# python-microscopy/ch-shrinkwrap

Measured on AMD Instinct MI355X. Metric: vertex-updates/s (force+CG step) + achieved HBM GB/s, 1M pts/200k verts, higher is better.
Workload: dtype f32; 1 GPU; BASELINE configs[2]: two-lobe vesicle (smooth union of two R=300 nm spheres), 1000000 localizations sigma=10 nm, 198812 vertices / 397620 faces, lams=[10], blocks of 5 iterations, fixed topology; localizations_per_gpu=1000000, vertices_per_gpu=198812, faces_per_gpu=397620, block=5, mode=single, parallelism=single GPU

## Files before the change

ch_shrinkwrap_amd/build.py:

```python
import glob
import os
import subprocess

HERE = os.path.dirname(os.path.abspath(__file__))
LIB = os.path.join(HERE, 'libnanowrap_hip.so')


def _csrc(name):
    return os.path.join(HERE, 'csrc', name)


def _include(name):
    return os.path.join(os.path.dirname(HERE), 'include', name)


HIPCC_FLAGS = ['-O3', '--offload-arch=gfx950', '-fPIC', '-shared', '-ffp-contract=off', '-munsafe-fp-atomics',
               '-fvisibility=hidden', '-Wall', '-Wno-unused-function']
_BASE = ['-O3', '--offload-arch=gfx950', '-fPIC', '-fvisibility=hidden']
_QUERY = _BASE + ['-ffp-contract=off', '-Wall', '-Wno-unused-function']
_BQ = [_csrc('nw_bq.h'), _csrc('nw_device.h')]

OBJ_MAIN, OBJ_HOLEPUNCH, OBJ_SURGERY, OBJ_BQ = _csrc('nanowrap.o'), _csrc('nw_holepunch.o'), _csrc('nw_surgery.o'), _csrc('nw_bq.o')
OBJ_ISOSURFACE = _csrc('nw_isosurface.o')
OBJ_EVALUATION = _csrc('nw_evaluation.o')
# ... 17 lines not shown
def needs_build():
    if not os.path.exists(LIB):
        return True
    t = os.path.getmtime(LIB)
    return any(os.path.getmtime(d) > t for d in DEPS)


def build_hip_library(force=False, verbose=False):
    if not force and not needs_build():
        return LIB
    hipcc = os.environ.get('HIPCC', '/opt/rocm/bin/hipcc')

    def run(cmd):
        if verbose:
            print(' '.join(cmd))
        subprocess.check_call(cmd)

    for src, obj, extra, flags in UNITS:
        if force or not os.path.exists(obj) or os.path.getmtime(obj) < max(os.path.getmtime(d) for d in [src] + extra):
            run([hipcc] + flags + ['-c', '-o', obj, src])
    check_kernel_budgets(verbose=verbose)
    run([hipcc, '--offload-arch=gfx950', '-fPIC', '-shared', '-o', LIB] + [obj for _, obj, _, _ in UNITS])
    return LIB


LLVM_BIN = os.environ.get('NW_LLVM_BIN', '/opt/rocm/lib/llvm/bin')
KERNEL_BUDGETS = {
    'k_nn_wave<false>':               (80, 10 * 1024),
    'k_attract':                      (72, 20 * 1024),
    'k_face_centroids':               (64, 8 * 1024),
    'k_centroid_scatter':             (64, 0),
    'k_scan_final':                   (64, 1024),
    'k_prior_ring':                   (128, 1024),
    'k_prior_directions':             (96, 1024),
    'k_subspace_point_sums':          (128, 1024),
    'k_solve_update':                 (128, 1024),
    'k_hp_empty_faces':               (64, 0),
    'k_hp_pair':                      (64, 8 * 1024),
    'k_hp_prism':                     (176, 0),
    'k_hp_cell_count':                (32, 0),
    'k_hp_scatter':                   (32, 0),
    'k_hp_bbox':                      (32, 0),
    'k_hp_cand_geom':                 (32, 0),
    'k_hp_pair_final':                (16, 0),
    'k_ws_init':                      (16, 0),
    'k_ws_hook':                      (32, 0),
    'k_ws_compress':                  (16, 0),
    'k_ws_number':                    (16, 0),
    'k_ws_stats':                     (64, 0),
    'k_ws_bbox_init':                 (16, 0),
    'k_ws_active':                    (16, 0),
    'k_ws_winding':                   (176, 0),
    'k_ws_lengths':                   (16, 0),
    'k_ws_hist':                      (16, 2048),
    'k_ws_pick':                      (32, 0),
    'k_ws_flag':                      (16, 0),
    'k_iso_count':                    (16, 16 * 1024),
    'k_iso_widen':                    (16, 0),
    'k_iso_smooth':                   (16, 0),
    'k_iso_hist':                     (16, 1024),
    'k_iso_pattern':                  (32, 0),
    'k_iso_compact':                  (16, 0),
    'k_iso_cell_counts':              (16, 0),
    'k_iso_vertices':                 (64, 0),
    'k_iso_quads':                    (32, 0),
    'k_ev_face_setup':                (64, 0),
    'k_ev_node_test':                 (32, 0),
    'k_ev_emit':                      (32, 0),
    'k_ev_bbox':                      (48, 0),
# ... 101 lines not shown
```

ch_shrinkwrap_amd/csrc/nanowrap.hip:

```cpp
#include <hip/hip_runtime.h>
#include <cstdio>
#include <cstdlib>
#include <cstring>
#include <cmath>
#include <string>
#include <vector>
#include <algorithm>
#include <chrono>
#include <thread>
#include <mutex>
#include <condition_variable>
#include <functional>
#include <atomic>
#include <memory>

#include "../../include/nanowrap.h"
#include "nw_kernels.h"

int nw_sort_pairs_u32(const unsigned *key_in, unsigned *key_out, const int *val_in, int *val_out, int n, int bits, hipStream_t stream);

static_assert(sizeof(NwIterLogDev) == sizeof(nw_iter_log), "device/host log record mismatch");
static_assert(SC_COUNT <= NW_N_SCALARS, "scalar slots");

#define NW_EXPORT extern "C" __attribute__((visibility("default")))
// ... 1524 lines not shown
        hipLaunchKernelGGL(k_nn_fixup, dim3(fb), dim3(NW_BLOCK), 0, ctx->stream, g, ctx->ambig_list.p, ctx->ambig_count.p, ctx->pts.p, ctx->cstart.p, ctx->cent.p,
                           ctx->cent_tmp.p, ctx->face.p, ctx->state.p, it, ctx->face_sorted ? ctx->face_orig.p : nullptr);
    }
    NW_HIP(hipGetLastError());
    return NW_OK;
}

static int iter_attract_parts(nw_ctx *ctx, int parts)
{
    if (ctx->begin_ops_pending) NW_TRY(enqueue_begin_ops(ctx));
    const int it = ctx->search_done;
    const int64_t N = ctx->N;
    const bool attract_rides = (parts & QP_NN) && (parts & QP_ATTRACT) && attract_in_nn() && fuse_fixup() && ctx->item_done.p != nullptr && ctx->face_warm && !ctx->handoff_off;
    bool rode = false;
    if (parts & (QP_GRID | QP_NN | QP_FIXUP)) NW_TRY(launch_query(ctx, it, parts & (QP_GRID | QP_NN | QP_FIXUP), true, attract_rides, &rode));
    if ((parts & QP_ATTRACT) && !rode) {
        StageScope s(ctx, ST_ATTRACT);
        hipLaunchKernelGGL(k_attract, dim3(attract_blocks(ctx)), dim3(NW_BLOCK), 0, ctx->stream, (int)N, ctx->pts.p, ctx->face.p, attract_args(ctx), ctx->state.p, it);
        ctx->attract_rows = attract_blocks(ctx);
    }
    NW_HIP(hipGetLastError());
    return NW_OK;
}

NW_EXPORT int nw_iter_attract(nw_ctx *ctx)
{
    if (!ctx || !ctx->in_search) return fail(ctx, NW_ERR_BADARG, "nw_iter_attract outside a search");
    if (ctx->have_boundary && ctx->pos_unpack_pending) { ctx->pos_unpack_pending = false; NW_TRY(halo_unpack(ctx, NW_ARR_POS)); }
    NW_TRY(iter_attract_parts(ctx, QP_ALL));
    if (ctx->have_boundary) NW_TRY(halo_pack(ctx, NW_ARR_VACC));
    return NW_OK;
}

NW_EXPORT int nw_iter_directions(nw_ctx *ctx)
{
    if (!ctx || !ctx->in_search) return fail(ctx, NW_ERR_BADARG, "nw_iter_directions outside a search");
    if (ctx->have_boundary) NW_TRY(halo_unpack(ctx, NW_ARR_VACC));
    const int it = ctx->search_done;
    const int n_search = (ctx->search_done == 0 || (ctx->search_flags & NW_FLAG_NO_LAST_STEP)) ? 2 : 3;
    {
        StageScope s(ctx, ST_PRIOR);
        const bool wfunc = (ctx->search_flags & NW_FLAG_WFUNC) != 0;
        if (wfunc)
            hipLaunchKernelGGL(k_vertex_area_weights, dim3(nblk(ctx->M)), dim3(NW_BLOCK), 0, ctx->stream, (int)ctx->M, ctx->NB, ctx->nbr.p, ctx->pos.p, ctx->wv.p, ctx->state.p, it);
        if (!ring_in_nn()) hipLaunchKernelGGL(k_prior_ring, dim3(nblk(ctx->M)), dim3(NW_BLOCK), 0, ctx->stream, ring_args(ctx), ctx->state.p, it);
        hipLaunchKernelGGL(k_prior_directions, dim3(prior_blocks(ctx)), dim3(NW_BLOCK), 0, ctx->stream, (int)ctx->M, ctx->ring4.p, ctx->ring_a.p, ctx->pos.p,
                           ctx->meshpos.p, ctx->nrm.p, ctx->vacc.p, ctx->S.p, ctx->fdef.p, ctx->pi.p, ctx->part_p.p, ctx->state.p, it, n_search,
                           ctx->acc_quantum, ctx->w_quantum, wfunc ? ctx->wv.p : nullptr, ctx->have_owned ? ctx->owned.p : nullptr);
    }
    {
        StageScope s(ctx, ST_AS);
        hipLaunchKernelGGL(k_subspace_point_sums, dim3(subspace_blocks(ctx)), dim3(NW_BLOCK), 0, ctx->stream, (int)ctx->N, (int)ctx->M, ctx->vidx.p, ctx->w.p, ctx->res.p,
                           ctx->mask.p, ctx->S.p, ctx->part_s.p, ctx->state.p, it, n_search);
        hipLaunchKernelGGL(k_reduce_scalars, dim3(3 * NW_SPARTS), dim3(NW_BLOCK), 0, ctx->stream, ctx->part_a.p, ctx->attract_rows, ctx->part_p.p, prior_blocks(ctx),
                           ctx->part_s.p, subspace_blocks(ctx), ctx->scalars.p, ctx->state.p, it);
    }
    NW_HIP(hipGetLastError());
    return NW_OK;
}

NW_EXPORT int nw_iter_update(nw_ctx *ctx)
{
    if (!ctx || !ctx->in_search) return fail(ctx, NW_ERR_BADARG, "nw_iter_update outside a search");
    if (ctx->search_done >= ctx->search_iters) return fail(ctx, NW_ERR_BADARG, "nw_iter_update: more iterations than announced");
    const int it = ctx->search_done;
    const int n_search = (ctx->search_done == 0 || (ctx->search_flags & NW_FLAG_NO_LAST_STEP)) ? 2 : 3;
    {
        StageScope s(ctx, ST_UPDATE);
        hipLaunchKernelGGL(k_solve_update, dim3(std::min(nblk(ctx->M), 512)), dim3(NW_BLOCK), 0, ctx->stream, (int)ctx->M, ctx->lam0, n_search, ctx->search_flags,
                           ctx->have_valid ? ctx->valid.p : nullptr, ctx->pos.p, ctx->meshpos.p, ctx->S.p, ctx->vacc.p, ctx->scalars.p, ctx->state.p,
                           ctx->logs.p + ctx->search_done, it, (ctx->direct_out && it == ctx->search_iters - 1) ? (float *)ctx->pin : nullptr);
    }
    NW_HIP(hipGetLastError());
    if (ctx->have_boundary) { NW_TRY(halo_pack(ctx, NW_ARR_POS)); ctx->pos_unpack_pending = true; }
    ctx->global_iter += 1;
    ctx->search_done += 1;
    return NW_OK;
}

static int write_back_impl(nw_ctx *ctx, float *contiguous, void *rows, int64_t row_stride_bytes);
static int ensure_staging(nw_ctx *ctx);
static void copy_out_staged(nw_ctx *ctx, float *contiguous, void *rows, int64_t row_stride_bytes);
static bool copy_out_chunks(nw_ctx *ctx, float *contiguous, void *rows, int64_t row_stride_bytes, int64_t slice_rows, int flag_base);

static int ensure_pin_log(nw_ctx *ctx, int n_records)
{
    const size_t log_bytes = (size_t)std::max(n_records, 1) * sizeof(nw_iter_log);
    if (ctx->pin_log_bytes < log_bytes + sizeof(NwDevState)) {
        if (ctx->pin_log) (void)hipHostFree(ctx->pin_log);
        ctx->pin_log = nullptr; ctx->pin_log_bytes = 0;
        NW_HIP(hipHostMalloc(&ctx->pin_log, 2 * log_bytes + sizeof(NwDevState), hipHostMallocDefault));
        ctx->pin_log_bytes = 2 * log_bytes + sizeof(NwDevState);
    }
    return NW_OK;
}

static bool spin_wait_on() { static const bool on = !(getenv("NW_SPIN_WAIT") && atoi(getenv("NW_SPIN_WAIT")) == 0); return on; }
static int enqueue_block_done(nw_ctx *ctx)
{
    ctx->done_launched = false;
    if (!spin_wait_on() || ctx->search_done <= 0) return NW_OK;
    NW_TRY(ensure_pin_log(ctx, ctx->search_iters));
    if (!ctx->pin_flag) {
        NW_HIP(hipHostMalloc((void **)&ctx->pin_flag, 64, hipHostMallocDefault));
        ctx->pin_flag[0] = 0;
        NW_HIP(ctx->done_count.ensure(1));
        NW_HIP(hipMemsetAsync(ctx->done_count.p, 0, sizeof(int), ctx->stream));
        ctx->done_expected = 0;
    }
    NwDevState *stp = (NwDevState *)((char *)ctx->pin_log + ctx->pin_log_bytes - sizeof(NwDevState));
// ... 274 lines not shown
    if (r == ncclSuccess) r = e;
    if (r != ncclSuccess) return fail(ctx, NW_ERR_HIP, std::string("ncclSend/ncclRecv: ") + (g_rccl.GetErrorString ? g_rccl.GetErrorString(r) : "error"));
    return NW_OK;
}

static int comm_after_attract(nw_ctx *ctx)
{
    if (!ctx->comm || !ctx->comm_mode) return NW_OK;
    if (ctx->comm_mode & NW_FLAG_COMM_REPLICATED) return comm_all_reduce_dev(ctx, ctx->vacc.p, (size_t)4 * ctx->M, ncclInt64, ncclSum);
    if ((ctx->comm_mode & NW_FLAG_COMM_HALO) && ctx->have_boundary && ctx->have_peers) {
        NW_TRY(px_exchange(ctx, false, 4, ncclInt64, 8));
        NW_TRY(px_stage(ctx, NW_ARR_VACC, 1));
        return px_exchange(ctx, true, 4, ncclFloat, 4);
    }
    if ((ctx->comm_mode & NW_FLAG_COMM_HALO) && ctx->have_boundary && ctx->hb_nslot > 0) return comm_all_reduce_dev(ctx, ctx->halo_acc.p, (size_t)4 * ctx->hb_nslot, ncclInt64, ncclSum);
    return NW_OK;
}
static int comm_after_directions(nw_ctx *ctx)
{
    if (!ctx->comm || !ctx->comm_mode) return NW_OK;
    const size_t n = (size_t)((ctx->comm_mode & NW_FLAG_COMM_REPLICATED) ? SC_NPOINT : SC_MAXD) * NW_SPARTS;
    return comm_all_reduce_dev(ctx, ctx->scalars.p, n, ncclDouble, ncclSum);
}
static int comm_after_update(nw_ctx *ctx)
{
    if (!ctx->comm || !ctx->comm_mode) return NW_OK;
    if ((ctx->comm_mode & NW_FLAG_COMM_HALO) && ctx->have_boundary && ctx->have_peers) return px_exchange(ctx, true, 3, ncclFloat, 4);
    if ((ctx->comm_mode & NW_FLAG_COMM_HALO) && ctx->have_boundary && ctx->hb_nslot > 0) return comm_all_reduce_dev(ctx, ctx->halo_rows.p, (size_t)3 * ctx->hb_nslot, ncclFloat, ncclSum);
    return NW_OK;
}

static int run_iteration(nw_ctx *ctx)
{
    int r = nw_iter_attract(ctx);
    if (r == NW_OK) r = comm_after_attract(ctx);
    if (r == NW_OK) r = nw_iter_directions(ctx);
    if (r == NW_OK) r = comm_after_directions(ctx);
    if (r == NW_OK) r = nw_iter_update(ctx);
    if (r == NW_OK) r = comm_after_update(ctx);
    return r;
}

NW_EXPORT int nw_comm_unique_id(uint8_t *out, int64_t nbytes)
{
    if (!out || nbytes < (int64_t)sizeof(ncclUniqueId)) return NW_ERR_BADARG;
    if (!g_rccl.load()) return NW_ERR_HIP;
    ncclUniqueId id;
    if (g_rccl.GetUniqueId(&id) != ncclSuccess) return NW_ERR_HIP;
    memcpy(out, &id, sizeof(id));
    return NW_OK;
}

NW_EXPORT int nw_comm_init(nw_ctx *ctx, const uint8_t *unique_id, int64_t nbytes, int rank, int nranks)
{
    if (!ctx) return NW_ERR_BADARG;
    NW_HIP(hipSetDevice(ctx->device));
    if (ctx->comm) {
        NW_HIP(hipStreamSynchronize(ctx->stream));
        for (auto &gph : ctx->graphs) if (gph.exec) { (void)hipGraphExecDestroy(gph.exec); gph.exec = nullptr; }
        (void)g_rccl.CommDestroy(ctx->comm);
        ctx->comm = nullptr; ctx->comm_rank = 0; ctx->comm_ranks = 1;
        ctx->comm_patterns.clear();
    }
    if (nranks <= 0) return NW_OK;
    if (!unique_id || nbytes < (int64_t)sizeof(ncclUniqueId) || rank < 0 || rank >= nranks) return fail(ctx, NW_ERR_BADARG, "nw_comm_init: unique id (nw_comm_unique_id of rank 0), 0 <= rank < nranks");
    (void)setenv("NCCL_GRAPH_REGISTER", "0", 0);
    if (!g_rccl.load()) return fail(ctx, NW_ERR_HIP, g_rccl.err);
    ncclUniqueId id;
    memcpy(&id, unique_id, sizeof(id));
    const ncclResult_t r = g_rccl.CommInitRank(&ctx->comm, nranks, id, rank);
    if (r != ncclSuccess) { ctx->comm = nullptr; return fail(ctx, NW_ERR_HIP, std::string("ncclCommInitRank: ") + (g_rccl.GetErrorString ? g_rccl.GetErrorString(r) : "error")); }
// ... 604 lines not shown
```

ch_shrinkwrap_amd/csrc/nw_kernels.h:

```cpp
#pragma once
#include "nw_device.h"

enum {
    SC_RES2 = 0,
    SC_C0 = 1,
    SC_SUMD = 2,
    SC_NPTS = 3,
    SC_HC = 4,
    SC_GC = 10,
    SC_STATUS = 13,
    SC_NPOINT = 14,
    SC_SS = 14,
    SC_SP = 20,
    SC_PP64 = 23,
    SC_PP32 = 24,
    SC_T = 25,
    SC_MAXD = 28,
    SC_COUNT = 29
};

#define NW_SPARTS 32

struct NwDevState {
    int stop_at;
// ... 388 lines not shown
        for (int j = 0; j < 3; ++j)
#pragma unroll
            for (int k = 0; k < 4; ++k) q[j][k] = 0ull;
        if (ok) {
            bool bad = false;
            nw_attract_point(A, i, pts[i], f_raw, v, q, red, dmax, bad);
            if (bad) atomicCAS(&st->status, 0, -3 );
        }
        const bool last_of_run = nw_run_sums(q, ok ? f_raw : -2 - (int)(threadIdx.x & 15));
        if (ok && last_of_run) nw_attract_scatter<NW_HT, NW_HT_BITS, NW_HT_PROBES>(A, v, q, s_key, s_val);
    }
    __syncthreads();
    {
        __shared__ double s_w[5 * 4];
        const int lane = threadIdx.x & 63, wv = threadIdx.x >> 6;
#pragma unroll
        for (int k = 0; k < 4; ++k) {
            const double sk = nw_wave_sum(red[k]);
            if (lane == 0) s_w[k * 4 + wv] = sk;
        }
#pragma unroll
        for (int off = 32; off > 0; off >>= 1) dmax = fmaxf(dmax, __shfl_xor(dmax, off, 64));
        if (lane == 0) s_w[16 + wv] = (double)dmax;
        __syncthreads();
        if (threadIdx.x < 4) A.part[(int64_t)blockIdx.x * 5 + threadIdx.x] = (s_w[threadIdx.x * 4 + 0] + s_w[threadIdx.x * 4 + 1]) + (s_w[threadIdx.x * 4 + 2] + s_w[threadIdx.x * 4 + 3]);
        else if (threadIdx.x == 4) A.part[(int64_t)blockIdx.x * 5 + 4] = fmax(fmax(s_w[16], s_w[17]), fmax(s_w[18], s_w[19]));
    }
    for (int t = threadIdx.x; t < NW_HT * 4; t += NW_BLOCK) {
        const int key = s_key[t >> 2];
        if (key >= 0) atomicAdd(reinterpret_cast<unsigned long long *>(A.vacc) + 4 * (int64_t)key + (t & 3), s_val[(t & 3) * NW_HT + (t >> 2)]);
    }
}

__global__ __launch_bounds__(NW_BLOCK) void k_prior_ring(const NwRingArgs R, const NwDevState *__restrict__ st, int it)
{
    if (st->iter_base + it >= st->stop_at) return;
    const int v = blockIdx.x * blockDim.x + threadIdx.x;
    if (v < R.M) nw_prior_ring_vertex(R, v);
}

__global__ __launch_bounds__(NW_BLOCK) void k_prior_directions(int M, const float4 *__restrict__ ring4, const double *__restrict__ ring_a, const float *__restrict__ pos,
                                                              const float *__restrict__ meshpos, const float *__restrict__ nrm,
                                                              const long long *__restrict__ vacc, float *__restrict__ S, float *__restrict__ fdef_out,
                                                              float *__restrict__ pi_out, double *__restrict__ part, NwDevState *__restrict__ st, int it, int n_search,
                                                              double q, double qw, const float *__restrict__ wv, const unsigned char *__restrict__ owned)
{
    if (st->iter_base + it >= st->stop_at) return;
    __shared__ double s_part[14 * 4];
    double red[14];
#pragma unroll
    for (int k = 0; k < 14; ++k) red[k] = 0.0;
    for (int v = blockIdx.x * blockDim.x + threadIdx.x; v < M; v += gridDim.x * blockDim.x) {
        const longlong2 a01 = *reinterpret_cast<const longlong2 *>(vacc + 4 * (int64_t)v), a23 = *reinterpret_cast<const longlong2 *>(vacc + 4 * (int64_t)v + 2);
        const float4 rg = ring4[v];
        const double asum = ring_a[v];
        const nw_f3u Nn = *reinterpret_cast<const nw_f3u *>(nrm + 3 * (int64_t)v);
        const nw_f3u Pm = *reinterpret_cast<const nw_f3u *>(meshpos + 3 * (int64_t)v);
        const nw_f3u Pf = *reinterpret_cast<const nw_f3u *>(pos + 3 * (int64_t)v);
        float *Srow = S + (int64_t)v * 9;
        const float s2c[3] = {n_search > 2 ? Srow[2] : 0.0f, n_search > 2 ? Srow[5] : 0.0f, n_search > 2 ? Srow[8] : 0.0f};
        const float lw = wv ? wv[v] : 1.0f;
        const bool mine = owned ? owned[v] != 0 : true;
        const float4 acc = make_float4((float)((double)a01.x * q), (float)((double)a01.y * q), (float)((double)a23.x * q), (float)((double)a23.y * qw));
        const float sw = acc.w;
        const float pi = sqrtf((sw * sw + sw * sw) + sw * sw);
        const float gate = fminf(pi * pi, 1.0f);
        pi_out[v] = pi;
        const int ms = __float_as_int(rg.w);
        double fd[3];
        if (ms > 0) {
            const double vcx = (double)rg.x / ms, vcy = (double)rg.y / ms, vcz = (double)rg.z / ms;
            const double alpha = (asum / ms) * (double)gate;
            fd[0] = vcx + alpha * (double)Nn.x; fd[1] = vcy + alpha * (double)Nn.y; fd[2] = vcz + alpha * (double)Nn.z;
        } else {
            fd[0] = Pm.x; fd[1] = Pm.y; fd[2] = Pm.z;
        }
        const float pf[3] = {Pf.x, Pf.y, Pf.z};
        const float s0[3] = {acc.x, acc.y, acc.z};
#pragma unroll
        for (int c = 0; c < 3; ++c) {
            double p64 = (double)pf[c] - fd[c];
            if (wv) p64 = p64 * (double)lw;
            const float p32 = (float)p64;
            const float s1 = wv ? -1.0f * (p32 * lw) : -1.0f * p32;
            float *row = Srow + 3 * c;
// ... 13 lines not shown
            red[7] += (double)l1 * p64;
            red[8] += (double)l2 * p64;
            red[9] += p64 * p64;
            red[10] += (double)p32 * (double)p32;
            red[11] += (double)s0[c] * s0[c];
            red[12] += (double)s0[c] * s1;
            red[13] += (double)s1 * s1;
        }
    }
    nw_block_sums_store<14>(red, part, s_part);
}

__global__ __launch_bounds__(NW_BLOCK) void k_vertex_area_weights(int M, int NB, const int *__restrict__ nbr, const float *__restrict__ f, float *__restrict__ wv,
                                                                 const NwDevState *__restrict__ st, int it)
{
    if (st->iter_base + it >= st->stop_at) return;
    const int i = blockIdx.x * blockDim.x + threadIdx.x;
    if (i >= M) return;
    const int *row = nbr + (int64_t)i * NB;
    float w = 0;
    for (int k = 0; k < NB; ++k) {
        const int n = row[k]; if (n == -1) break;
        float d2 = 0;
        for (int j = 0; j < 3; ++j) { const float dd = f[3 * n + j] - f[3 * i + j]; d2 += dd * dd; }
        w += d2;
    }
    wv[i] = (w > 0) ? (float)(1.0 / (double)sqrtf(w + 1)) : 0.0f;
}

#define NW_SUBSPACE_PPT 4

__global__ __launch_bounds__(NW_BLOCK) void k_subspace_point_sums(int N, int M, const int *__restrict__ vidx, const float *__restrict__ w, const float *__restrict__ res,
                                                                 const unsigned char *__restrict__ mask, const float *__restrict__ S, double *__restrict__ part,
                                                                 const NwDevState *__restrict__ st, int it, int n_search)
{
    if (st->iter_base + it >= st->stop_at) return;
    __shared__ double s_w[9 * 4];
    const int blk = nw_xcd_remap(blockIdx.x, (N + NW_BLOCK * NW_SUBSPACE_PPT - 1) / (NW_BLOCK * NW_SUBSPACE_PPT));
    double red[9];
#pragma unroll
    for (int k = 0; k < 9; ++k) red[k] = 0.0;
    nw_i3u vi[NW_SUBSPACE_PPT];
    nw_f3u wj[NW_SUBSPACE_PPT], rr[NW_SUBSPACE_PPT];
    unsigned msk[NW_SUBSPACE_PPT];
#pragma unroll
    for (int p = 0; p < NW_SUBSPACE_PPT; ++p) {
        const int64_t i = blk < 0 ? (int64_t)N : ((int64_t)blk * NW_SUBSPACE_PPT + p) * NW_BLOCK + threadIdx.x;
        const int64_t ic = i < N ? i : 0;
        vi[p] = *reinterpret_cast<const nw_i3u *>(vidx + 3 * ic);
        wj[p] = *reinterpret_cast<const nw_f3u *>(w + 3 * ic);
        rr[p] = *reinterpret_cast<const nw_f3u *>(res + 3 * ic);
        const unsigned m = mask[ic];
        msk[p] = i < N ? m : 0u;
    }
#pragma unroll
    for (int h = 0; h < NW_SUBSPACE_PPT; h += 2) {
        float row[2][3][9];
#pragma unroll
        for (int q = 0; q < 2; ++q)
#pragma unroll
            for (int j = 0; j < 3; ++j) {
                const unsigned v = min((unsigned)vi[h + q][j], (unsigned)(M - 1));
                const float *src = S + (int64_t)v * 9;
                const nw_f4u a = *reinterpret_cast<const nw_f4u *>(src), b = *reinterpret_cast<const nw_f4u *>(src + 4);
                row[q][j][0] = a.x; row[q][j][1] = a.y; row[q][j][2] = a.z; row[q][j][3] = a.w;
                row[q][j][4] = b.x; row[q][j][5] = b.y; row[q][j][6] = b.z; row[q][j][7] = b.w;
                row[q][j][8] = src[8];
            }
#pragma unroll
        for (int q = 0; q < 2; ++q) {
// ... 102 lines not shown
#pragma unroll
        for (int r = k + 1; r < N; ++r) {
            const bool sw = fabsf(A[r][k]) > mx;
            mx = sw ? fabsf(A[r][k]) : mx;
#pragma unroll
            for (int c = 0; c < 4; ++c) { const float t = A[k][c]; A[k][c] = sw ? A[r][c] : t; A[r][c] = sw ? t : A[r][c]; }
        }
        singular = singular || !(mx > 0.0f);
#pragma unroll
        for (int r = k + 1; r < N; ++r) {
            const float l = A[r][k] / A[k][k];
#pragma unroll
            for (int c = k; c < 4; ++c) A[r][c] = A[r][c] - l * A[k][c];
        }
    }
    float x[3] = {0.0f, 0.0f, 0.0f};
#pragma unroll
    for (int k = N - 1; k >= 0; --k) {
        float sacc = A[k][3];
#pragma unroll
        for (int c = k + 1; c < N; ++c) sacc = sacc - A[k][c] * x[c];
        x[k] = sacc / A[k][k];
    }
    o.singular = singular ? 1 : 0;
#pragma unroll
    for (int k = 0; k < 3; ++k) o.c[k] = singular ? 0.0f : x[k];
}

struct NwIterLogDev {
    double test, res_norm, prefs_norm, cpred, wpred, c[3], H[9], G[3], mean_dist, max_dist;
    int n_search, nn_max_ring, status, executed;
};

__global__ __launch_bounds__(NW_BLOCK) void k_solve_update(int M, float lam, int n_search, unsigned flags, const unsigned char *__restrict__ valid,
                                                          float *__restrict__ pos, float *__restrict__ meshpos, float *__restrict__ S, long long *__restrict__ vacc,
                                                          const double *__restrict__ sc_parts, NwDevState *__restrict__ st,
                                                          NwIterLogDev *__restrict__ logrec, int it, float *__restrict__ host_out)
{
    if (st->iter_base + it >= st->stop_at) return;
    __shared__ NwSolve s_sol;
    __shared__ double s_sc[SC_COUNT];
    const int stride = (int)(gridDim.x * blockDim.x);
    const int v0 = blockIdx.x * blockDim.x + threadIdx.x;
    constexpr int NPRE = 2;
    float pre_row[NPRE][9], pre_pos[NPRE][3];
    unsigned char pre_ok[NPRE];
#pragma unroll
    for (int u = 0; u < NPRE; ++u) {
        const int v = v0 + u * stride;
        const int vc = v < M ? v : 0;
        const float *src = S + (int64_t)vc * 9;
        const nw_f4u a = *reinterpret_cast<const nw_f4u *>(src), b = *reinterpret_cast<const nw_f4u *>(src + 4);
        pre_row[u][0] = a.x; pre_row[u][1] = a.y; pre_row[u][2] = a.z; pre_row[u][3] = a.w;
        pre_row[u][4] = b.x; pre_row[u][5] = b.y; pre_row[u][6] = b.z; pre_row[u][7] = b.w;
        pre_row[u][8] = src[8];
        const nw_f3u p3 = *reinterpret_cast<const nw_f3u *>(pos + 3 * (int64_t)vc);
        pre_pos[u][0] = p3.x; pre_pos[u][1] = p3.y; pre_pos[u][2] = p3.z;
        pre_ok[u] = *(valid ? valid + vc : &nw_byte_one);
    }
    if (threadIdx.x < SC_COUNT) {
        double pp[NW_SPARTS];
#pragma unroll
        for (int b = 0; b < NW_SPARTS; ++b) pp[b] = sc_parts[threadIdx.x * NW_SPARTS + b];
        double t = 0.0;
        if (threadIdx.x == SC_MAXD) {
#pragma unroll
            for (int b = 0; b < NW_SPARTS; ++b) t = fmax(t, pp[b]);
        } else {
#pragma unroll
            for (int b = 0; b < NW_SPARTS; ++b) t += pp[b];
        }
        s_sc[threadIdx.x] = t;
    }
    __syncthreads();
    const double *sc = s_sc;
    if (threadIdx.x == 0) { if (n_search > 2) nw_solve_small<3>(sc, lam, s_sol); else nw_solve_small<2>(sc, lam, s_sol); }
    __syncthreads();
    const NwSolve sol = s_sol;
    const bool failed = st->status != 0 || sc[SC_STATUS] > 0.0;
    const bool go = !sol.singular && !failed;
    auto update_vertex = [&](int v, const float (&row)[9], const float (&f0)[3], bool ok) {
        float fn[3];
#pragma unroll
        for (int c = 0; c < 3; ++c) {
            float step = row[3 * c + 0] * sol.c[0];
            step = step + row[3 * c + 1] * sol.c[1];
            if (n_search > 2) step = step + row[3 * c + 2] * sol.c[2];
            fn[c] = f0[c] + step;
            if ((flags & 1u) && !(fn[c] > 0.0f)) fn[c] = fn[c] * 0.0f;
        }
        if (go) {
            if (!(flags & 2u)) {
#pragma unroll
                for (int c = 0; c < 3; ++c) S[(int64_t)v * 9 + 3 * c + 2] = fn[c] - f0[c];
            }
            nw_f3u o; o.x = fn[0]; o.y = fn[1]; o.z = fn[2];
// ... 31 lines not shown
        double cHc = 0, cG = 0, cHwc = 0, cGw = 0;
#pragma unroll
        for (int r = 0; r < 3; ++r) {
            if (r < n_search) {
                cG += (double)sol.c[r] * sol.G[r];
                cGw += (double)sol.c[r] * (-sc[SC_SP + r]);
#pragma unroll
                for (int c = 0; c < 3; ++c)
                    if (c < n_search) {
                        cHc += (double)sol.c[r] * sol.H[3 * r + c] * sol.c[c];
                        cHwc += (double)sol.c[r] * (double)(float)sc[SC_SS + nw_tri(r, c)] * sol.c[c];
                    }
            }
        }
        L.cpred = sc[SC_C0] + cHc - cG;
        L.wpred = sc[SC_PP64] + cHwc - cGw;
        for (int k = 0; k < 3; ++k) { L.c[k] = sol.c[k]; L.G[k] = sol.G[k]; }
        for (int k = 0; k < 9; ++k) L.H[k] = sol.H[k];
        L.mean_dist = sc[SC_NPTS] > 0 ? sc[SC_SUMD] / sc[SC_NPTS] : 0.0;
        L.max_dist = sc[SC_MAXD];
        L.n_search = n_search;
        L.nn_max_ring = st->nn_max_ring;
        if (sol.singular) atomicCAS(&st->status, 0, -4 );
        if (sc[SC_STATUS] > 0.0) atomicCAS(&st->status, 0, -8 );
        L.status = st->status;
        L.executed = (failed || sol.singular) ? 0 : 1;
        *logrec = L;
        float a = st->tests[1], b = st->tests[2];
        st->tests[0] = a; st->tests[1] = b; st->tests[2] = test;
        st->ntests += 1;
        if (st->ntests >= 3 && (test < b) && (b < a) && (a < 1e-6f)) st->stop_at = st->iter_base + it + 1;
        if (st->status != 0) st->stop_at = st->iter_base + it + 1;
    }
}

template <int NV, int NT, int MAXCOL, int MAXSLOT>
__device__ __forceinline__ void nw_reduce_columns(const double *__restrict__ part, int nblk, double *s_acc , double *__restrict__ sc, int slot0, int bid)
{
    static_assert(NT % NV == 0 && NT <= NW_BLOCK, "thread count must be a multiple of the row length");
    const int t = threadIdx.x;
    const int per = (nblk + NW_SPARTS - 1) / NW_SPARTS;
    const int r0 = min(bid * per, nblk), r1 = min(r0 + per, nblk);
    const double *__restrict__ p = part + (int64_t)r0 * NV;
    const int64_t total = (int64_t)(r1 - r0) * NV;
    double a0 = 0.0, a1 = 0.0, a2 = 0.0, a3 = 0.0;
    if (t < NT) {
        int64_t e = t;
        if (MAXCOL >= 0 && t % NV == MAXCOL) {
            for (; e < total; e += NT) a0 = fmax(a0, p[e]);
            s_acc[t] = a0;
        } else {
            for (; e + 3 * NT < total; e += 4 * NT) { a0 += p[e]; a1 += p[e + NT]; a2 += p[e + 2 * NT]; a3 += p[e + 3 * NT]; }
            for (; e < total; e += NT) a0 += p[e];
            s_acc[t] = (a0 + a1) + (a2 + a3);
        }
    }
    __syncthreads();
    if (t < NV) {
        double s = 0.0;
        if (MAXCOL >= 0 && t == MAXCOL) { for (int k = t; k < NT; k += NV) s = fmax(s, s_acc[k]); }
        else { for (int k = t; k < NT; k += NV) s += s_acc[k]; }
        sc[((MAXCOL >= 0 && t == MAXCOL) ? MAXSLOT : slot0 + t) * NW_SPARTS + bid] = s;
    }
    __syncthreads();
}

__global__ __launch_bounds__(NW_BLOCK) void k_reduce_scalars(const double *__restrict__ part_a, int nblk_a, const double *__restrict__ part_p, int nblk_p,
                                                            const double *__restrict__ part_s, int nblk_s, double *__restrict__ sc,
                                                            const NwDevState *__restrict__ st, int it)
{
    if (st->iter_base + it >= st->stop_at) return;
    __shared__ double s_acc[NW_BLOCK];
    const int table = (int)blockIdx.x / NW_SPARTS, bid = (int)blockIdx.x % NW_SPARTS;
    if (table == 0 && threadIdx.x == 0) sc[SC_STATUS * NW_SPARTS + bid] = (bid == 0 && st->status != 0) ? 1.0 : 0.0;
    if (table == 0) nw_reduce_columns<5, 255, 4, SC_MAXD>(part_a, nblk_a, s_acc, sc, SC_RES2, bid);
    else if (table == 1) nw_reduce_columns<9, 252, -1, 0>(part_s, nblk_s, s_acc, sc, SC_HC, bid);
    else nw_reduce_columns<14, 252, -1, 0>(part_p, nblk_p, s_acc, sc, SC_SS, bid);
}

__global__ void k_apply_A(int N, const int *__restrict__ perm, const int *__restrict__ vidx, const float *__restrict__ w, const float *__restrict__ x, float *__restrict__ y)
{
    const int i = blockIdx.x * blockDim.x + threadIdx.x;
    if (i >= N) return;
    const int o = perm[i];
#pragma unroll
    for (int c = 0; c < 3; ++c) {
        float a = 0.0f;
#pragma unroll
        for (int j = 0; j < 3; ++j) a = a + x[3 * vidx[3 * i + j] + c] * w[3 * i + j];
        y[3 * o + c] = a;
    }
}

__global__ void k_apply_At(int N, const int *__restrict__ perm, const int *__restrict__ vidx, const float *__restrict__ w, const float *__restrict__ r, float *__restrict__ z)
{
    const int i = blockIdx.x * blockDim.x + threadIdx.x;
    if (i >= N) return;
// ... 485 lines not shown
```

ch_shrinkwrap_amd/mesh_conj_grad.py:

```python
import ctypes
import os
import numpy as np

from . import _lib as nw


class NativeContext(object):

    def __init__(self, device=0, stream=None):
        self.L = nw.load()
        self.h = ctypes.c_void_p()
        code = self.L.nw_create(int(device), ctypes.byref(self.h))
        if code != nw.NW_OK:
            raise nw.NanoWrapError(code, 'nw_create failed (is a MI355X visible? HIP extension present?)')
        if stream is not None:
            self.check(self.L.nw_set_stream(self.h, ctypes.c_void_p(int(stream))))
        self.device = int(device)
        self.points_key = None
        self._keep = []

    def check(self, code):
        nw.check(self.L, self.h, code)

    def close(self):
# ... 208 lines not shown
        if self.mesh.__dict__.get('_rows_pending') is not None:
            self._flush_rows()
        return self._vertices_view

    def _flush_rows(self):
        self.mesh.__dict__['_rows_pending'] = None
        self._native.check(self._L.nw_synchronize(self._h))

    def synchronize(self):
        self._flush_rows()

    def _consume_logs(self, logs, executed):
        self.loopcount = executed
        for i in range(executed):
            L = logs[i]
            self.tests.append(np.float32(L.test))
            self.ress.append(np.float32(L.res_norm))
            self.prefs.append(np.array([L.prefs_norm], np.float32))
            self.cpred = np.float32(L.cpred)
            self.wpreds = [np.float64(L.wpred)]
            self.nn_max_ring = max(self.nn_max_ring, int(L.nn_max_ring))
            self.mean_dist = float(L.mean_dist)
            self.max_dist = max(getattr(self, 'max_dist', 0.0), float(L.max_dist))
        if executed:
            self._raw_logs.append((logs, executed))

    @property
    def iter_logs(self):
        for logs, executed in self._raw_logs:
            for i in range(executed):
                L = logs[i]
                self._iter_logs.append(dict(test=L.test, res_norm=L.res_norm, prefs_norm=L.prefs_norm, cpred=L.cpred, wpred=L.wpred,
                                            c=np.array(L.c[:]), H=np.array(L.H[:]).reshape(3, 3), G=np.array(L.G[:]),
                                            mean_dist=L.mean_dist, n_search=int(L.n_search), nn_max_ring=int(L.nn_max_ring)))
        self._raw_logs = []
        return self._iter_logs

    def _result_buffer(self):
        import sys
        pool = self._fs_pool
        for i in range(len(pool)):
            if sys.getrefcount(pool[i]) <= 2 and pool[i].shape == (self.M, 3):
                return pool[i]
        b = np.empty((self.M, 3), np.float32)
        pool.append(b)
        if len(pool) > 3:
            del pool[0]
        return b

    def _finish(self):
        out = self._result_buffer()
        posv = self._records()['position']
        stride = posv.strides[0]
        if posv.dtype == np.float32 and posv.strides[1] == 4 and stride >= 12:
            self._native.check(self._L.nw_write_back(self._h, nw.ptr(out), ctypes.c_void_p(posv.ctypes.data), stride))
        else:
            self._native.check(self._L.nw_write_back(self._h, nw.ptr(out), None, 0))
            np.copyto(posv, out, where=self._mesh_vertex_mask[:, None])
        self.fs = out
        self.f = self.fs.ravel()
        self.mesh._initialize_curvature_vectors()

    def _get(self, what, shape, dtype):
        if what in self._cache:
            return self._cache[what]
        a = np.empty(shape, dtype)
        self._native.check(self._L.nw_get(self._h, what, nw.ptr(a), a.nbytes))
# ... 146 lines not shown
```

Measured before the change: 777.1 million vertex-updates/s.

## Fold scalar reductions into prior, subspace and solve kernels to drop reduce launch

Removes the separate k_reduce_scalars launch per iteration. The attract-partial reduction now runs in extra blocks appended to k_prior_directions, the prior-partial reduction in extra blocks appended to k_subspace_point_sums, and the subspace-partial reduction is done redundantly inside every k_solve_update block through shared memory. The goal is to save one kernel launch and its dependency bubble per iteration. In exchange each solve block repeats the row-sum work and uses about 64 KB more shared memory, which can lower occupancy. The path is gated by an environment variable, a row-count threshold and single-device mode.

```diff
diff --git a/ch_shrinkwrap_amd/build.py b/ch_shrinkwrap_amd/build.py
--- a/ch_shrinkwrap_amd/build.py
+++ b/ch_shrinkwrap_amd/build.py
@@ -73,9 +73,10 @@
     'k_centroid_scatter':             (64, 0),
     'k_scan_final':                   (64, 1024),
     'k_prior_ring':                   (128, 1024),
-    'k_prior_directions':             (96, 1024),
-    'k_subspace_point_sums':          (128, 1024),
-    'k_solve_update':                 (128, 1024),
+    'k_prior_directions':             (96, 2048),
+    'k_subspace_point_sums':          (128, 2048),
+    'k_solve_update<false>':          (128, 1024),
+    'k_solve_update<true>':           (128, 64 * 1024),
     'k_hp_empty_faces':               (64, 0),
     'k_hp_pair':                      (64, 8 * 1024),
     'k_hp_prism':                     (176, 0),
diff --git a/ch_shrinkwrap_amd/csrc/nanowrap.hip b/ch_shrinkwrap_amd/csrc/nanowrap.hip
--- a/ch_shrinkwrap_amd/csrc/nanowrap.hip
+++ b/ch_shrinkwrap_amd/csrc/nanowrap.hip
@@ -1580,50 +1580,83 @@
     return NW_OK;
 }
 
-NW_EXPORT int nw_iter_directions(nw_ctx *ctx)
-{
-    if (!ctx || !ctx->in_search) return fail(ctx, NW_ERR_BADARG, "nw_iter_directions outside a search");
+enum { RM_LAUNCH = 0, RM_INLINE = 1 };
+#define NW_REDUCE_INLINE_ROWS_DEFAULT 256
+static int reduce_inline_rows()
+{
+    static const int rows = getenv("NW_REDUCE_INLINE_ROWS") ? std::max(0, std::min(NW_SOLVE_SUMS_MAX_ROWS, atoi(getenv("NW_REDUCE_INLINE_ROWS")))) : NW_REDUCE_INLINE_ROWS_DEFAULT;
+    return rows;
+}
+static int reduce_mode(const nw_ctx *ctx)
+{
+    static const bool on = !(getenv("NW_REDUCE_INLINE") && atoi(getenv("NW_REDUCE_INLINE")) == 0);
+    if (!on || (ctx->comm && ctx->comm_mode) || ctx->have_boundary) return RM_LAUNCH;
+    return subspace_blocks(ctx) <= reduce_inline_rows() ? RM_INLINE : RM_LAUNCH;
+}
+
+static int iter_directions(nw_ctx *ctx, int rmode)
+{
     if (ctx->have_boundary) NW_TRY(halo_unpack(ctx, NW_ARR_VACC));
     const int it = ctx->search_done;
     const int n_search = (ctx->search_done == 0 || (ctx->search_flags & NW_FLAG_NO_LAST_STEP)) ? 2 : 3;
+    const bool appended = rmode != RM_LAUNCH;
     {
         StageScope s(ctx, ST_PRIOR);
         const bool wfunc = (ctx->search_flags & NW_FLAG_WFUNC) != 0;
         if (wfunc)
             hipLaunchKernelGGL(k_vertex_area_weights, dim3(nblk(ctx->M)), dim3(NW_BLOCK), 0, ctx->stream, (int)ctx->M, ctx->NB, ctx->nbr.p, ctx->pos.p, ctx->wv.p, ctx->state.p, it);
         if (!ring_in_nn()) hipLaunchKernelGGL(k_prior_ring, dim3(nblk(ctx->M)), dim3(NW_BLOCK), 0, ctx->stream, ring_args(ctx), ctx->state.p, it);
-        hipLaunchKernelGGL(k_prior_directions, dim3(prior_blocks(ctx)), dim3(NW_BLOCK), 0, ctx->stream, (int)ctx->M, ctx->ring4.p, ctx->ring_a.p, ctx->pos.p,
+        hipLaunchKernelGGL(k_prior_directions, dim3(prior_blocks(ctx) + (appended ? NW_SPARTS : 0)), dim3(NW_BLOCK), 0, ctx->stream, (int)ctx->M, ctx->ring4.p, ctx->ring_a.p, ctx->pos.p,
                            ctx->meshpos.p, ctx->nrm.p, ctx->vacc.p, ctx->S.p, ctx->fdef.p, ctx->pi.p, ctx->part_p.p, ctx->state.p, it, n_search,
-                           ctx->acc_quantum, ctx->w_quantum, wfunc ? ctx->wv.p : nullptr, ctx->have_owned ? ctx->owned.p : nullptr);
+                           ctx->acc_quantum, ctx->w_quantum, wfunc ? ctx->wv.p : nullptr, ctx->have_owned ? ctx->owned.p : nullptr,
+                           prior_blocks(ctx), ctx->part_a.p, ctx->attract_rows, ctx->scalars.p);
     }
     {
         StageScope s(ctx, ST_AS);
-        hipLaunchKernelGGL(k_subspace_point_sums, dim3(subspace_blocks(ctx)), dim3(NW_BLOCK), 0, ctx->stream, (int)ctx->N, (int)ctx->M, ctx->vidx.p, ctx->w.p, ctx->res.p,
-                           ctx->mask.p, ctx->S.p, ctx->part_s.p, ctx->state.p, it, n_search);
-        hipLaunchKernelGGL(k_reduce_scalars, dim3(3 * NW_SPARTS), dim3(NW_BLOCK), 0, ctx->stream, ctx->part_a.p, ctx->attract_rows, ctx->part_p.p, prior_blocks(ctx),
-                           ctx->part_s.p, subspace_blocks(ctx), ctx->scalars.p, ctx->state.p, it);
+        hipLaunchKernelGGL(k_subspace_point_sums, dim3(subspace_blocks(ctx) + (appended ? NW_SPARTS : 0)), dim3(NW_BLOCK), 0, ctx->stream, (int)ctx->N, (int)ctx->M, ctx->vidx.p, ctx->w.p, ctx->res.p,
+                           ctx->mask.p, ctx->S.p, ctx->part_s.p, ctx->state.p, it, n_search, subspace_blocks(ctx), ctx->part_p.p, prior_blocks(ctx), ctx->scalars.p);
+        if (rmode != RM_INLINE)
+            hipLaunchKernelGGL(k_reduce_scalars, dim3(3 * NW_SPARTS), dim3(NW_BLOCK), 0, ctx->stream, ctx->part_a.p, ctx->attract_rows, ctx->part_p.p, prior_blocks(ctx),
+                               ctx->part_s.p, subspace_blocks(ctx), ctx->scalars.p, ctx->state.p, it);
     }
     NW_HIP(hipGetLastError());
     return NW_OK;
 }
 
-NW_EXPORT int nw_iter_update(nw_ctx *ctx)
-{
-    if (!ctx || !ctx->in_search) return fail(ctx, NW_ERR_BADARG, "nw_iter_update outside a search");
+NW_EXPORT int nw_iter_directions(nw_ctx *ctx)
+{
+    if (!ctx || !ctx->in_search) return fail(ctx, NW_ERR_BADARG, "nw_iter_directions outside a search");
+    return iter_directions(ctx, RM_LAUNCH);
+}
+
+static int iter_update(nw_ctx *ctx, int rmode)
+{
     if (ctx->search_done >= ctx->search_iters) return fail(ctx, NW_ERR_BADARG, "nw_iter_update: more iterations than announced");
     const int it = ctx->search_done;
     const int n_search = (ctx->search_done == 0 || (ctx->search_flags & NW_FLAG_NO_LAST_STEP)) ? 2 : 3;
     {
         StageScope s(ctx, ST_UPDATE);
-        hipLaunchKernelGGL(k_solve_update, dim3(std::min(nblk(ctx->M), 512)), dim3(NW_BLOCK), 0, ctx->stream, (int)ctx->M, ctx->lam0, n_search, ctx->search_flags,
-                           ctx->have_valid ? ctx->valid.p : nullptr, ctx->pos.p, ctx->meshpos.p, ctx->S.p, ctx->vacc.p, ctx->scalars.p, ctx->state.p,
-                           ctx->logs.p + ctx->search_done, it, (ctx->direct_out && it == ctx->search_iters - 1) ? (float *)ctx->pin : nullptr);
+        float *const host_out = (ctx->direct_out && it == ctx->search_iters - 1) ? (float *)ctx->pin : nullptr;
+        if (rmode == RM_INLINE)
+            hipLaunchKernelGGL(k_solve_update<true>, dim3(std::min(nblk(ctx->M), 512)), dim3(NW_BLOCK), 0, ctx->stream, (int)ctx->M, ctx->lam0, n_search, ctx->search_flags,
+                               ctx->have_valid ? ctx->valid.p : nullptr, ctx->pos.p, ctx->meshpos.p, ctx->S.p, ctx->vacc.p, ctx->scalars.p, ctx->state.p,
+                               ctx->logs.p + ctx->search_done, it, host_out, ctx->part_s.p, subspace_blocks(ctx));
+        else
+            hipLaunchKernelGGL(k_solve_update<false>, dim3(std::min(nblk(ctx->M), 512)), dim3(NW_BLOCK), 0, ctx->stream, (int)ctx->M, ctx->lam0, n_search, ctx->search_flags,
+                               ctx->have_valid ? ctx->valid.p : nullptr, ctx->pos.p, ctx->meshpos.p, ctx->S.p, ctx->vacc.p, ctx->scalars.p, ctx->state.p,
+                               ctx->logs.p + ctx->search_done, it, host_out, nullptr, 0);
     }
     NW_HIP(hipGetLastError());
     if (ctx->have_boundary) { NW_TRY(halo_pack(ctx, NW_ARR_POS)); ctx->pos_unpack_pending = true; }
     ctx->global_iter += 1;
     ctx->search_done += 1;
     return NW_OK;
+}
+
+NW_EXPORT int nw_iter_update(nw_ctx *ctx)
+{
+    if (!ctx || !ctx->in_search) return fail(ctx, NW_ERR_BADARG, "nw_iter_update outside a search");
+    return iter_update(ctx, RM_LAUNCH);
 }
 
 static int write_back_impl(nw_ctx *ctx, float *contiguous, void *rows, int64_t row_stride_bytes);
@@ -1964,11 +1997,13 @@
 
 static int run_iteration(nw_ctx *ctx)
 {
+    if (!ctx || !ctx->in_search) return fail(ctx, NW_ERR_BADARG, "iteration outside a search");
+    const int rmode = reduce_mode(ctx);
     int r = nw_iter_attract(ctx);
     if (r == NW_OK) r = comm_after_attract(ctx);
-    if (r == NW_OK) r = nw_iter_directions(ctx);
+    if (r == NW_OK) r = iter_directions(ctx, rmode);
     if (r == NW_OK) r = comm_after_directions(ctx);
-    if (r == NW_OK) r = nw_iter_update(ctx);
+    if (r == NW_OK) r = iter_update(ctx, rmode);
     if (r == NW_OK) r = comm_after_update(ctx);
     return r;
 }
diff --git a/ch_shrinkwrap_amd/csrc/nw_kernels.h b/ch_shrinkwrap_amd/csrc/nw_kernels.h
--- a/ch_shrinkwrap_amd/csrc/nw_kernels.h
+++ b/ch_shrinkwrap_amd/csrc/nw_kernels.h
@@ -444,6 +444,37 @@
     }
 }
 
+template <int NV, int NT, int MAXCOL, int MAXSLOT>
+__device__ __forceinline__ void nw_reduce_columns(const double *__restrict__ part, int nblk, double *s_acc , double *__restrict__ sc, int slot0, int bid)
+{
+    static_assert(NT % NV == 0 && NT <= NW_BLOCK, "thread count must be a multiple of the row length");
+    const int t = threadIdx.x;
+    const int per = (nblk + NW_SPARTS - 1) / NW_SPARTS;
+    const int r0 = min(bid * per, nblk), r1 = min(r0 + per, nblk);
+    const double *__restrict__ p = part + (int64_t)r0 * NV;
+    const int64_t total = (int64_t)(r1 - r0) * NV;
+    double a0 = 0.0, a1 = 0.0, a2 = 0.0, a3 = 0.0;
+    if (t < NT) {
+        int64_t e = t;
+        if (MAXCOL >= 0 && t % NV == MAXCOL) {
+            for (; e < total; e += NT) a0 = fmax(a0, p[e]);
+            s_acc[t] = a0;
+        } else {
+            for (; e + 3 * NT < total; e += 4 * NT) { a0 += p[e]; a1 += p[e + NT]; a2 += p[e + 2 * NT]; a3 += p[e + 3 * NT]; }
+            for (; e < total; e += NT) a0 += p[e];
+            s_acc[t] = (a0 + a1) + (a2 + a3);
+        }
+    }
+    __syncthreads();
+    if (t < NV) {
+        double s = 0.0;
+        if (MAXCOL >= 0 && t == MAXCOL) { for (int k = t; k < NT; k += NV) s = fmax(s, s_acc[k]); }
+        else { for (int k = t; k < NT; k += NV) s += s_acc[k]; }
+        sc[((MAXCOL >= 0 && t == MAXCOL) ? MAXSLOT : slot0 + t) * NW_SPARTS + bid] = s;
+    }
+    __syncthreads();
+}
+
 __global__ __launch_bounds__(NW_BLOCK) void k_prior_ring(const NwRingArgs R, const NwDevState *__restrict__ st, int it)
 {
     if (st->iter_base + it >= st->stop_at) return;
@@ -455,14 +486,21 @@
                                                               const float *__restrict__ meshpos, const float *__restrict__ nrm,
                                                               const long long *__restrict__ vacc, float *__restrict__ S, float *__restrict__ fdef_out,
                                                               float *__restrict__ pi_out, double *__restrict__ part, NwDevState *__restrict__ st, int it, int n_search,
-                                                              double q, double qw, const float *__restrict__ wv, const unsigned char *__restrict__ owned)
+                                                              double q, double qw, const float *__restrict__ wv, const unsigned char *__restrict__ owned,
+                                                              int nb_vertex, const double *__restrict__ part_a, int nblk_a, double *__restrict__ sc)
 {
     if (st->iter_base + it >= st->stop_at) return;
-    __shared__ double s_part[14 * 4];
+    __shared__ double s_part[NW_BLOCK];
+    if ((int)blockIdx.x >= nb_vertex) {
+        const int bid = (int)blockIdx.x - nb_vertex;
+        if (threadIdx.x == 0) sc[SC_STATUS * NW_SPARTS + bid] = (bid == 0 && st->status != 0) ? 1.0 : 0.0;
+        nw_reduce_columns<5, 255, 4, SC_MAXD>(part_a, nblk_a, s_part, sc, SC_RES2, bid);
+        return;
+    }
     double red[14];
 #pragma unroll
     for (int k = 0; k < 14; ++k) red[k] = 0.0;
-    for (int v = blockIdx.x * blockDim.x + threadIdx.x; v < M; v += gridDim.x * blockDim.x) {
+    for (int v = blockIdx.x * blockDim.x + threadIdx.x; v < M; v += nb_vertex * blockDim.x) {
         const longlong2 a01 = *reinterpret_cast<const longlong2 *>(vacc + 4 * (int64_t)v), a23 = *reinterpret_cast<const longlong2 *>(vacc + 4 * (int64_t)v + 2);
         const float4 rg = ring4[v];
         const double asum = ring_a[v];
@@ -542,10 +580,15 @@
 
 __global__ __launch_bounds__(NW_BLOCK) void k_subspace_point_sums(int N, int M, const int *__restrict__ vidx, const float *__restrict__ w, const float *__restrict__ res,
                                                                  const unsigned char *__restrict__ mask, const float *__restrict__ S, double *__restrict__ part,
-                                                                 const NwDevState *__restrict__ st, int it, int n_search)
+                                                                 const NwDevState *__restrict__ st, int it, int n_search,
+                                                                 int nb_point, const double *__restrict__ part_p, int nblk_p, double *__restrict__ sc)
 {
     if (st->iter_base + it >= st->stop_at) return;
-    __shared__ double s_w[9 * 4];
+    __shared__ double s_w[NW_BLOCK];
+    if ((int)blockIdx.x >= nb_point) {
+        nw_reduce_columns<14, 252, -1, 0>(part_p, nblk_p, s_w, sc, SC_SS, (int)blockIdx.x - nb_point);
+        return;
+    }
     const int blk = nw_xcd_remap(blockIdx.x, (N + NW_BLOCK * NW_SUBSPACE_PPT - 1) / (NW_BLOCK * NW_SUBSPACE_PPT));
     double red[9];
 #pragma unroll
@@ -714,10 +757,67 @@
     int n_search, nn_max_ring, status, executed;
 };
 
+#define NW_SOLVE_SUMS_MAX_ROWS (2 * 28 * NW_SPARTS)
+
+template <int NJ>
+__device__ __forceinline__ void nw_solve_row_values(const double *__restrict__ part, int nblk, int per, int nact, double *s_acc)
+{
+    constexpr int NV = 9, NT = 252;
+    const int nvirt = NW_SPARTS * nact;
+    const int64_t last = (int64_t)nblk * NV - 1;
+#pragma unroll 4
+    for (int i = threadIdx.x; i < nvirt; i += NW_BLOCK) {
+        const int b = i / nact, t = i - b * nact;
+        const int r0 = min(b * per, nblk), r1 = min(r0 + per, nblk);
+        const int total = (r1 - r0) * NV;
+        const int64_t base = (int64_t)r0 * NV + t;
+        static_assert(NJ <= 2, "more elements per thread bring nw_reduce_columns' four chains into play");
+        double x[2] = {0.0, 0.0};
+#pragma unroll
+        for (int j = 0; j < NJ; ++j) {
+            const double v = part[min(base + j * NT, last)];
+            x[j] = (t + j * NT < total) ? v : 0.0;
+        }
+        s_acc[b * NT + t] = (0.0 + x[0]) + x[1];
+    }
+}
+
+__device__ __forceinline__ void nw_solve_row_sums(const double *__restrict__ part, int nblk, double *s_acc)
+{
+    constexpr int NV = 9, NT = 252;
+    const int per = (nblk + NW_SPARTS - 1) / NW_SPARTS;
+    const int nact = min(NT, per * NV);
+    if (per * NV <= NT) nw_solve_row_values<1>(part, nblk, per, nact, s_acc);
+    else nw_solve_row_values<2>(part, nblk, per, nact, s_acc);
+    __syncthreads();
+    const int nk = nact / NV;
+    double r[2] = {0.0, 0.0};
+    static_assert(NW_SPARTS * NV <= 2 * NW_BLOCK, "two sums per thread");
+#pragma unroll
+    for (int u = 0; u < 2; ++u) {
+        const int i = threadIdx.x + u * NW_BLOCK;
+        if (i < NW_SPARTS * NV) {
+            const double *a = s_acc + (i / NV) * NT + i % NV;
+            double s = 0.0;
+            for (int k = 0; k < nk; ++k) s += a[k * NV];
+            r[u] = s;
+        }
+    }
+    __syncthreads();
+#pragma unroll
+    for (int u = 0; u < 2; ++u) {
+        const int i = threadIdx.x + u * NW_BLOCK;
+        if (i < NW_SPARTS * NV) s_acc[(i % NV) * NW_SPARTS + i / NV] = r[u];
+    }
+    __syncthreads();
+}
+
+template <bool SUMS>
 __global__ __launch_bounds__(NW_BLOCK) void k_solve_update(int M, float lam, int n_search, unsigned flags, const unsigned char *__restrict__ valid,
                                                           float *__restrict__ pos, float *__restrict__ meshpos, float *__restrict__ S, long long *__restrict__ vacc,
-                                                          const double *__restrict__ sc_parts, NwDevState *__restrict__ st,
-                                                          NwIterLogDev *__restrict__ logrec, int it, float *__restrict__ host_out)
+                                                          double *__restrict__ sc_parts, NwDevState *__restrict__ st,
+                                                          NwIterLogDev *__restrict__ logrec, int it, float *__restrict__ host_out,
+                                                          const double *__restrict__ part_s, int nblk_s)
 {
     if (st->iter_base + it >= st->stop_at) return;
     __shared__ NwSolve s_sol;
@@ -740,10 +840,17 @@
         pre_pos[u][0] = p3.x; pre_pos[u][1] = p3.y; pre_pos[u][2] = p3.z;
         pre_ok[u] = *(valid ? valid + vc : &nw_byte_one);
     }
+    __shared__ double s_rows[SUMS ? NW_SPARTS * 252 : 1];
+    const double *s_hc = s_rows;
+    if (SUMS) {
+        nw_solve_row_sums(part_s, nblk_s, s_rows);
+        if (blockIdx.x == 0) for (int i = threadIdx.x; i < 9 * NW_SPARTS; i += NW_BLOCK) sc_parts[SC_HC * NW_SPARTS + i] = s_hc[i];
+    }
     if (threadIdx.x < SC_COUNT) {
+        const bool own = SUMS && threadIdx.x >= SC_HC && threadIdx.x < SC_HC + 9;
         double pp[NW_SPARTS];
 #pragma unroll
-        for (int b = 0; b < NW_SPARTS; ++b) pp[b] = sc_parts[threadIdx.x * NW_SPARTS + b];
+        for (int b = 0; b < NW_SPARTS; ++b) pp[b] = own ? s_hc[(threadIdx.x - SC_HC) * NW_SPARTS + b] : sc_parts[threadIdx.x * NW_SPARTS + b];
         double t = 0.0;
         if (threadIdx.x == SC_MAXD) {
 #pragma unroll
@@ -841,37 +948,6 @@
         if (st->ntests >= 3 && (test < b) && (b < a) && (a < 1e-6f)) st->stop_at = st->iter_base + it + 1;
         if (st->status != 0) st->stop_at = st->iter_base + it + 1;
     }
-}
-
-template <int NV, int NT, int MAXCOL, int MAXSLOT>
-__device__ __forceinline__ void nw_reduce_columns(const double *__restrict__ part, int nblk, double *s_acc , double *__restrict__ sc, int slot0, int bid)
-{
-    static_assert(NT % NV == 0 && NT <= NW_BLOCK, "thread count must be a multiple of the row length");
-    const int t = threadIdx.x;
-    const int per = (nblk + NW_SPARTS - 1) / NW_SPARTS;
-    const int r0 = min(bid * per, nblk), r1 = min(r0 + per, nblk);
-    const double *__restrict__ p = part + (int64_t)r0 * NV;
-    const int64_t total = (int64_t)(r1 - r0) * NV;
-    double a0 = 0.0, a1 = 0.0, a2 = 0.0, a3 = 0.0;
-    if (t < NT) {
-        int64_t e = t;
-        if (MAXCOL >= 0 && t % NV == MAXCOL) {
-            for (; e < total; e += NT) a0 = fmax(a0, p[e]);
-            s_acc[t] = a0;
-        } else {
-            for (; e + 3 * NT < total; e += 4 * NT) { a0 += p[e]; a1 += p[e + NT]; a2 += p[e + 2 * NT]; a3 += p[e + 3 * NT]; }
-            for (; e < total; e += NT) a0 += p[e];
-            s_acc[t] = (a0 + a1) + (a2 + a3);
-        }
-    }
-    __syncthreads();
-    if (t < NV) {
-        double s = 0.0;
-        if (MAXCOL >= 0 && t == MAXCOL) { for (int k = t; k < NT; k += NV) s = fmax(s, s_acc[k]); }
-        else { for (int k = t; k < NT; k += NV) s += s_acc[k]; }
-        sc[((MAXCOL >= 0 && t == MAXCOL) ? MAXSLOT : slot0 + t) * NW_SPARTS + bid] = s;
-    }
-    __syncthreads();
 }
 
 __global__ __launch_bounds__(NW_BLOCK) void k_reduce_scalars(const double *__restrict__ part_a, int nblk_a, const double *__restrict__ part_p, int nblk_p,
diff --git a/ch_shrinkwrap_amd/mesh_conj_grad.py b/ch_shrinkwrap_amd/mesh_conj_grad.py
--- a/ch_shrinkwrap_amd/mesh_conj_grad.py
+++ b/ch_shrinkwrap_amd/mesh_conj_grad.py
@@ -264,7 +264,7 @@
                 L = logs[i]
                 self._iter_logs.append(dict(test=L.test, res_norm=L.res_norm, prefs_norm=L.prefs_norm, cpred=L.cpred, wpred=L.wpred,
                                             c=np.array(L.c[:]), H=np.array(L.H[:]).reshape(3, 3), G=np.array(L.G[:]),
-                                            mean_dist=L.mean_dist, n_search=int(L.n_search), nn_max_ring=int(L.nn_max_ring)))
+                                            mean_dist=L.mean_dist, max_dist=L.max_dist, n_search=int(L.n_search), nn_max_ring=int(L.nn_max_ring)))
         self._raw_logs = []
         return self._iter_logs
 
```

After: 761.8 million vertex-updates/s. 2.0% lower.
